# eps696/aphantasia

Hardware: AMD Instinct MI355X
Metric: optimization steps/sec @1280x720 ViT-B/32 samples=200 (higher is better)
Workload: dtype f16 (MFMA operands, fp32 accumulate; fp32 residual stream / LayerNorm / softmax statistics / synth / sampler / loss / Adam)

## Files before the change

### aphantasia_amd/_ffi.py

```python
import ctypes
import os
from ctypes import POINTER, c_char_p, c_float, c_int, c_size_t, c_void_p

import torch

HERE = os.path.dirname(os.path.abspath(__file__))
LIB_PATH = os.path.join(HERE, 'libaphantasia_hip.so')

APH_OUT_NCHW_RAW, APH_OUT_NCHW_NORM, APH_OUT_PATCH_F16, APH_GRAD_PATCH_F16, APH_OUT_PATCH_F16_HILO, APH_OUT_PATCH_F32 = 0, 1, 2, 3, 4, 5
APH_AUG_STRIDE = 16
APH_TF_FAST, APH_TF_CUSTOM, APH_TF_ELASTIC = 0, 1, 2
SIM_TYPES = {'cossim': 0, 'cos': 0, None: 0, 'mix': 1, 'ang': 2, 'dot': 3}


class SampleGeom(ctypes.Structure):
    _fields_ = [(n, c_int) for n in ('H', 'W', 'Hp', 'Wp', 'py0', 'px0', 'S', 'size', 'patch')]


_PROTOTYPES = {
    'aph_version': (c_int, []),
    'aph_last_error': (c_char_p, []),
    'aph_synth_plan_create': (c_int, [c_int, c_int, c_int, POINTER(c_void_p)]),
    'aph_synth_plan_destroy': (c_int, [c_void_p]),
    'aph_synth_fft_fwd': (c_int, [c_void_p, c_void_p, c_void_p, c_void_p, c_float, POINTER(c_float), c_int, c_void_p, c_void_p, c_void_p]),
# ... 5 lines not shown
    'aph_synth_stats': (c_int, [c_void_p, c_void_p, c_void_p]),
    'aph_synth_set_stats': (c_int, [c_void_p, c_void_p, c_void_p]),
    'aph_synth_plan_describe': (c_int, [c_void_p, POINTER(c_int)]),
    'aph_idwt_coarse_levels': (c_int, [POINTER(c_int), POINTER(c_int), c_int, c_int]),
    'aph_rgb_priors_ws_bytes': (c_size_t, []),
    'aph_rgb_sharp': (c_int, [c_void_p, c_int, c_int, c_float, c_void_p, c_void_p, c_void_p, c_void_p]),
    'aph_rgb_priors': (c_int, [c_void_p, c_int, c_int, c_float, c_float, c_float, c_void_p, c_void_p, c_void_p, c_void_p]),
    'aph_cppn_param_count': (c_size_t, [c_int, c_int, c_int]),
    'aph_cppn_ws_bytes': (c_size_t, [c_int, c_int, c_int, c_int, c_int]),
    'aph_cppn_fwd': (c_int, [c_void_p, c_int, c_int, c_int, c_void_p, c_void_p, c_int, c_int, c_void_p, c_void_p, c_void_p]),
    'aph_cppn_bwd': (c_int, [c_void_p, c_int, c_int, c_int, c_void_p, c_void_p, c_int, c_int, c_void_p, c_float, c_void_p, c_void_p, c_void_p, c_void_p]),
    'aph_idwt_level_fwd': (c_int, [c_void_p, c_int, c_int, c_void_p, c_int, c_int, c_int, c_void_p, c_void_p, c_int, c_float, c_void_p, c_void_p]),
    'aph_idwt_fwd': (c_int, [c_void_p, c_void_p, c_void_p, c_void_p, c_void_p, c_int, c_int, c_void_p, c_void_p, c_int, c_void_p, c_void_p]),
    'aph_idwt_bwd': (c_int, [c_void_p, c_void_p, c_void_p, c_void_p, c_int, c_int, c_void_p, c_void_p, c_int, c_void_p, c_void_p, c_void_p, c_void_p]),
    'aph_idwt_level_bwd': (c_int, [c_void_p, c_int, c_int, c_int, c_void_p, c_void_p, c_int, c_float, c_void_p, c_int, c_int, c_void_p, c_void_p]),
    'aph_sample_ws_bytes': (c_size_t, [POINTER(SampleGeom), c_int]),
    'aph_sample_fwd': (c_int, [POINTER(SampleGeom), c_void_p, c_void_p, c_void_p, c_void_p, c_void_p, c_int, c_void_p]),
    'aph_sample_bwd': (c_int, [POINTER(SampleGeom), c_void_p, c_float, c_void_p, c_void_p, c_void_p, c_void_p, c_int, c_void_p]),
    'aph_sample_ws_bytes_tf': (c_size_t, [POINTER(SampleGeom), c_int]),
    'aph_sample_fwd_tf': (c_int, [POINTER(SampleGeom), c_int, c_void_p, c_void_p, c_void_p, c_void_p, c_void_p, c_void_p, c_int, c_void_p]),
    'aph_sample_bwd_tf': (c_int, [POINTER(SampleGeom), c_int, c_void_p, c_float, c_void_p, c_void_p, c_void_p, c_void_p, c_void_p, c_int, c_void_p]),
    'aph_triangle_blur': (c_int, [c_void_p, c_int, c_int, c_int, c_int, c_float, c_float, c_void_p, c_void_p]),
    'aph_resize_bicubic': (c_int, [c_void_p, c_int, c_int, c_int, c_void_p, c_int, c_int, c_void_p]),
    'aph_flip_w': (c_int, [c_void_p, c_void_p, c_int, c_int, c_int, c_void_p, c_void_p]),
    'aph_grid_warp': (c_int, [c_void_p, c_void_p, c_int, c_int, c_int, c_float, c_float, c_float, c_float, c_float, c_void_p, c_void_p, c_void_p]),
    'aph_attn_test': (c_int, [c_void_p, c_void_p, c_void_p, c_void_p, c_void_p, c_void_p, c_int, c_int, c_int, c_int, c_void_p]),
    'aph_attn_f32_test': (c_int, [c_void_p, c_void_p, c_void_p, c_void_p, c_void_p, c_void_p, c_int, c_int, c_int, c_int, c_void_p]),
    'aph_attn_causal_f32_test': (c_int, [c_void_p, c_void_p, c_void_p, c_int, c_int, c_int, c_void_p]),
    'aph_text_create': (c_int, [c_int, c_int, c_int, c_int, c_int, c_int, c_int, POINTER(c_void_p)]),
    'aph_text_destroy': (c_int, [c_void_p]),
    'aph_text_workspace_bytes': (c_size_t, [c_void_p]),
    'aph_text_set_weight': (c_int, [c_void_p, c_char_p, c_void_p, c_size_t]),
    'aph_text_forward': (c_int, [c_void_p, c_void_p, c_int, c_void_p, c_void_p]),
    'aph_lpips_create': (c_int, [POINTER(c_int), c_int, c_int, POINTER(c_void_p)]),
    'aph_lpips_destroy': (c_int, [c_void_p]),
    'aph_lpips_workspace_bytes': (c_size_t, [c_void_p]),
    'aph_lpips_set_weight': (c_int, [c_void_p, c_char_p, c_void_p, c_size_t]),
    'aph_lpips_set_target': (c_int, [c_void_p, c_void_p, c_int, c_int, c_void_p]),
    'aph_lpips_value_grad': (c_int, [c_void_p, c_void_p, c_void_p, c_void_p, c_void_p, c_void_p]),
    'aph_lpips_value_grad_half': (c_int, [c_void_p, c_void_p, c_void_p, c_void_p, c_void_p, c_void_p]),
    'aph_lpips_pack_test': (c_int, [c_void_p, c_int, c_int, c_int, c_void_p, c_size_t]),
    'aph_lpips_conv_test': (c_int, [c_void_p, c_int, c_int, c_int, c_void_p, c_int, c_void_p, c_int, c_void_p, c_void_p, c_void_p, c_int, c_int, c_void_p]),
    'aph_lpips_pool_test': (c_int, [c_void_p, c_int, c_int, c_int, c_void_p, c_void_p, c_void_p, c_void_p]),
    'aph_lpips_head_test': (c_int, [c_void_p, c_void_p, c_void_p, c_int, c_int, c_float, c_void_p, c_void_p, c_void_p, c_void_p, c_void_p]),
    'aph_lpips_resize_test': (c_int, [c_void_p, c_int, c_int, c_void_p, c_int, c_void_p]),
    'aph_depth_create': (c_int, [c_int, c_int, c_int, c_int, POINTER(c_int), POINTER(c_int), c_int, c_int, c_int, c_int, c_int, POINTER(c_void_p)]),
    'aph_depth_destroy': (c_int, [c_void_p]),
    'aph_depth_workspace_bytes': (c_size_t, [c_void_p]),
    'aph_depth_set_weight': (c_int, [c_void_p, c_char_p, c_void_p, c_size_t]),
    'aph_depth_set_pos_embed': (c_int, [c_void_p, c_int, c_int, c_void_p, c_size_t]),
    'aph_depth_forward': (c_int, [c_void_p, c_void_p, c_int, c_int, c_int, c_int, c_void_p, c_void_p]),
    'aph_depth_attn_test': (c_int, [c_void_p, c_void_p, c_int, c_int, c_int, c_void_p]),
    'aph_depth_conv_test': (c_int, [c_void_p, c_int, c_int, c_int, c_void_p, c_int, c_void_p, c_int, c_int, c_void_p, c_void_p, c_int, c_int, c_void_p, c_void_p,
                                    c_void_p]),
    'aph_depth_gemm_test': (c_int, [c_void_p, c_int, c_void_p, c_int, c_int, c_int, c_void_p, c_void_p, c_void_p]),
    'aph_depth_convt_test': (c_int, [c_void_p, c_int, c_int, c_int, c_int, c_void_p, c_int, c_int, c_void_p, c_void_p, c_void_p, c_void_p]),
    'aph_depth_resize_test': (c_int, [c_void_p, c_int, c_int, c_int, c_int, c_void_p, c_int, c_int, c_void_p]),
    'aph_depth_gelu_gemm_test': (c_int, [c_void_p, c_void_p, c_int, c_int, c_int, c_void_p, c_void_p, c_void_p]),
    'aph_frame_affine': (c_int, [c_void_p, c_int, c_int, c_int, POINTER(c_float), c_void_p, c_void_p]),
    'aph_patchify_f16': (c_int, [c_void_p, c_int, c_int, c_int, c_void_p, c_void_p]),
    'aph_patchify_f16_hilo': (c_int, [c_void_p, c_int, c_int, c_int, c_void_p, c_void_p]),
    'aph_patchify_f32': (c_int, [c_void_p, c_int, c_int, c_int, c_void_p, c_void_p]),
    'aph_unpatchify_f32': (c_int, [c_void_p, c_int, c_int, c_int, c_float, c_void_p, c_void_p]),
    'aph_patch_row_elems': (c_int, [c_int]),
    'aph_patchify_f16_win': (c_int, [c_void_p, c_int, c_int, c_int, c_int, c_void_p, c_void_p]),
    'aph_unpatchify_f32_win': (c_int, [c_void_p, c_int, c_int, c_int, c_int, c_float, c_void_p, c_void_p]),
    'aph_vit_create': (c_int, [c_int, c_int, c_int, c_int, c_int, c_int, c_int, POINTER(c_void_p)]),
    'aph_vit_destroy': (c_int, [c_void_p]),
    'aph_vit_workspace_bytes': (c_size_t, [c_void_p]),
    'aph_vit_set_weight': (c_int, [c_void_p, c_char_p, c_void_p, c_size_t]),
    'aph_vit_forward': (c_int, [c_void_p, c_void_p, c_int, c_void_p, c_void_p]),
    'aph_vit_forward_hilo': (c_int, [c_void_p, c_void_p, c_int, c_void_p, c_void_p]),
    'aph_vit_enable_hilo': (c_int, [c_void_p]),
    'aph_vit_enable_f32': (c_int, [c_void_p]),
    'aph_vit_forward_f32': (c_int, [c_void_p, c_void_p, c_int, c_void_p, c_void_p]),
    'aph_vit_backward_f32': (c_int, [c_void_p, c_void_p, c_int, c_void_p, c_float, c_void_p]),
    'aph_vit_backward': (c_int, [c_void_p, c_void_p, c_int, c_void_p, c_float, c_void_p]),
    'aph_vit_backward_h': (c_int, [c_void_p, c_void_p, c_int, c_void_p, c_float, c_void_p]),
    'aph_vit_profile': (c_int, [c_void_p, c_int]),
    'aph_vit_profile_read': (c_int, [c_void_p, c_void_p, c_void_p, c_void_p]),
    'aph_gemm_set_mfma32': (c_int, [c_int]),
    'aph_vit_set_fuse_ln': (c_int, [c_int]),
    'aph_crop_adjoint_set_gather': (c_int, [c_int]),
    'aph_crop_adjoint_set_shape': (c_int, [c_int, c_int, c_int, c_int, c_int]),
    'aph_vit_set_grad_stream_f16': (c_int, [c_int]),
    'aph_gemm_set_ws_min_tiles': (c_int, [c_int]),
    'aph_gemm_set_ws_pgroup': (c_int, [c_int]),
    'aph_gemm_set_rs': (c_int, [c_int]),
    'aph_mfma_rate': (c_int, [c_int, c_int, c_void_p, c_void_p, c_void_p]),
    'aph_gemm_rs_probe': (c_int, [c_void_p, c_void_p, c_int, c_int, c_int, c_void_p, c_int, c_void_p, c_void_p]),
    'aph_gemm_ws_probe': (c_int, [c_void_p, c_void_p, c_int, c_int, c_int, c_void_p, c_void_p, c_void_p, c_int, c_void_p, c_void_p]),
    'aph_gemm_f32_test': (c_int, [c_void_p, c_int, c_int, c_void_p, c_int, c_int, c_int, c_int, c_void_p, c_int, c_void_p, c_void_p, c_int, c_void_p, c_size_t, c_void_p]),
    'aph_gemm_f16': (c_int, [c_void_p, c_void_p, c_int, c_int, c_int, c_void_p, c_void_p]),
    'aph_gemm_f16_ld': (c_int, [c_void_p, c_int, c_void_p, c_int, c_int, c_int, c_int, c_void_p, c_int, c_void_p]),
    'aph_gemm_f16_epi_test': (c_int, [c_void_p, c_int, c_void_p, c_int, c_int, c_int, c_int, c_void_p, c_int, c_void_p, c_void_p, c_void_p, c_float, c_int,
                                      c_int, c_int, c_int, c_void_p, c_size_t, c_int, c_void_p]),
    'aph_ln_test': (c_int, [c_int, c_int, c_int, c_int, c_int, c_int, c_int, c_void_p, c_void_p, c_void_p, c_void_p, c_void_p, c_void_p, c_void_p,
                            c_void_p, c_void_p, c_void_p, c_void_p, c_void_p, c_void_p, c_void_p]),
    'aph_sim_loss': (c_int, [c_void_p, c_int, c_int, c_void_p, c_void_p, POINTER(c_float), c_int, c_int, c_int, c_int, c_int, c_float, c_float, c_void_p, c_void_p, c_void_p, c_void_p]),
    'aph_axpy_f32': (c_int, [c_void_p, c_void_p, c_float, c_size_t, c_void_p]),
    'aph_rgb_to_u8': (c_int, [c_void_p, c_int, c_int, c_float, c_void_p, c_void_p]),
    'aph_linear_head': (c_int, [c_void_p, c_int, c_int, c_void_p, c_float, c_float, c_float, c_float, c_void_p, c_void_p, c_void_p]),
    'aph_comm_unique_id': (c_int, [c_void_p]),
    'aph_comm_init': (c_int, [c_int, c_int, c_void_p, POINTER(c_void_p)]),
    'aph_allreduce_f32': (c_int, [c_void_p, c_void_p, c_size_t, c_void_p]),
    'aph_comm_ranks': (c_int, [c_void_p, POINTER(c_int)]),
    'aph_comm_destroy': (c_int, [c_void_p]),
    'aph_adam_step': (c_int, [c_void_p, c_void_p, c_void_p, c_void_p, c_void_p, c_void_p, c_int, c_size_t, c_void_p]),
    'aph_adam_step_guarded': (c_int, [c_void_p, c_void_p, c_void_p, c_void_p, c_void_p, c_void_p, c_int, c_size_t, c_void_p, c_void_p]),
}

EXPORTS = tuple(_PROTOTYPES)

class Library:

    def __init__(self, path):
        if not os.path.isfile(path):
            raise RuntimeError(
                "aphantasia_amd: HIP library not found at %s -- build it with "
                "`python -c 'import __graft_entry__ as g; g.build()'` (hipcc, gfx950). "
                "There is no CPU fallback." % path)
        self.path = path
        self.cdll = ctypes.CDLL(path)
        for name, (res, args) in _PROTOTYPES.items():
            fn = getattr(self.cdll, name)
            fn.restype = res
            fn.argtypes = args

    def last_error(self):
        return (self.cdll.aph_last_error() or b'').decode(errors='replace')

    def call(self, name, *args):
        rc = getattr(self.cdll, name)(*args)
        if rc < 0:
            raise RuntimeError('%s failed (%d): %s' % (name, rc, self.last_error()))
        return rc


_lib = None


def lib():
    global _lib
    if _lib is None:
        import torch
        if torch.cuda.is_available():
            torch.cuda.init()
            torch.empty(1, device='cuda')
        _lib = Library(LIB_PATH)
    return _lib


def ptr(t):
    return c_void_p(t.data_ptr()) if t is not None else c_void_p(0)


def floats(seq):
    if seq is None:
        return None
    arr = (c_float * len(seq))(*[float(v) for v in seq])
    return arr
```

### aphantasia_amd/csrc/sampler.hip

```cpp
#include <cstring>
#include <cstdlib>
#include <type_traits>

#include "sampler_layout.h"
#include "sampler_crop.h"
#include "sampler_crop_adjoint.h"
#include "sampler_warp.h"
#include "sampler_kornia.h"

namespace aph {

struct Nchw { int s, c, i, j; };
__device__ __forceinline__ Nchw nchw_of(size_t idx, int R) {
  return Nchw{(int)(idx / ((size_t)3 * R * R)), (int)((idx / ((size_t)R * R)) % 3), (int)((idx / R) % R), (int)(idx % R)};
}

__global__ void patchify_kernel(const float* __restrict__ x, half_t* __restrict__ out, int S, int R, int p, int hilo) {
  const size_t n = (size_t)S * 3 * R * R;
  const Layout<APH_OUT_PATCH_F16> L(R, p);
  for (size_t idx = (size_t)blockIdx.x * blockDim.x + threadIdx.x; idx < n; idx += (size_t)gridDim.x * blockDim.x) {
    const Nchw e = nchw_of(idx, R);
    const size_t o = L.index(e.s, e.c, e.i, e.j);
    const half_t h = (half_t)x[idx];
    if (!hilo) { out[o] = h; continue; }
// ... 1 lines not shown
    out[q] = h;
    out[q + L.patch_elems()] = (half_t)(x[idx] - (float)h);
  }
}
__global__ void patchify_f32_kernel(const float* __restrict__ x, float* __restrict__ out, int S, int R, int p) {
  const size_t n = (size_t)S * 3 * R * R;
  for (size_t idx = (size_t)blockIdx.x * blockDim.x + threadIdx.x; idx < n; idx += (size_t)gridDim.x * blockDim.x) {
    const Nchw e = nchw_of(idx, R);
    out[patch_index(e.s, e.c, e.i, e.j, R, p)] = x[idx];
  }
}
__global__ void unpatchify_kernel(const float* __restrict__ g, float* __restrict__ out, int S, int R, int p, float gscale) {
  const size_t n = (size_t)S * 3 * R * R;
  for (size_t idx = (size_t)blockIdx.x * blockDim.x + threadIdx.x; idx < n; idx += (size_t)gridDim.x * blockDim.x) {
    const Nchw e = nchw_of(idx, R);
    out[idx] = g[patch_index(e.s, e.c, e.i, e.j, R, p)] * gscale;
  }
}


__global__ void patchify_win_kernel(const float* __restrict__ x, half_t* __restrict__ out, int S, int Rs, int R, int p, int kp) {
  const int gp = R / p, k3 = 3 * p * p;
  const size_t n = (size_t)S * gp * gp * kp;
  for (size_t idx = (size_t)blockIdx.x * blockDim.x + threadIdx.x; idx < n; idx += (size_t)gridDim.x * blockDim.x) {
    const size_t row = idx / kp;
    const int k = (int)(idx - row * kp);
    float v = 0.f;
    if (k < k3) {
      const int s = (int)(row / ((size_t)gp * gp)), pr = (int)(row - (size_t)s * gp * gp), py = pr / gp, px = pr - py * gp;
      const int pix = k / 3, c = k - pix * 3, iy = pix / p, ix = pix - iy * p;
      v = x[(((size_t)s * 3 + c) * Rs + (py * p + iy)) * Rs + (px * p + ix)];
    }
    out[idx] = (half_t)v;
  }
}
__global__ void unpatchify_win_kernel(const float* __restrict__ g, float* __restrict__ out, int S, int Rs, int R, int p, int kp, float gscale) {
  const int gp = R / p;
  const size_t n = (size_t)S * 3 * Rs * Rs;
  for (size_t idx = (size_t)blockIdx.x * blockDim.x + threadIdx.x; idx < n; idx += (size_t)gridDim.x * blockDim.x) {
    const Nchw e = nchw_of(idx, Rs);
    float v = 0.f;
    if (e.i < R && e.j < R) {
      const int py = e.i / p, px = e.j / p, iy = e.i - py * p, ix = e.j - px * p;
      v = g[(((size_t)e.s * gp + py) * gp + px) * kp + (iy * p + ix) * 3 + e.c] * gscale;
    }
    out[idx] = v;
  }
}

}

using namespace aph;

static Geom to_geom(const aph_sample_geom* g) { return Geom{g->H, g->W, g->Hp, g->Wp, g->py0, g->px0, g->S, g->size, g->patch}; }

static int check_geom(const aph_sample_geom* g, int out_mode, const char* who, int max_mode = 2) {
  if (!g) return aph_fail(APH_ERR_ARG, "%s: null geometry", who);
  if (out_mode == APH_OUT_PATCH_F16_HILO && max_mode == 2) max_mode = APH_OUT_PATCH_F16_HILO;
  if (out_mode == APH_OUT_PATCH_F32) max_mode = APH_OUT_PATCH_F32;
  if (g->S < 1 || g->size < 1 || g->H < 1 || g->W < 1 || g->Hp < g->H || g->Wp < g->W)
    return aph_fail(APH_ERR_ARG, "%s: bad geometry S=%d size=%d H=%d W=%d Hp=%d Wp=%d", who, g->S, g->size, g->H, g->W, g->Hp, g->Wp);
  if (out_mode < 0 || out_mode > max_mode || (out_mode == APH_GRAD_PATCH_F16 && max_mode != APH_GRAD_PATCH_F16))
    return aph_fail(APH_ERR_ARG, "%s: bad out_mode %d", who, out_mode);
  if (out_mode >= APH_OUT_PATCH_F16 && (g->patch < 1 || g->size % g->patch || (g->patch & (g->patch - 1))))
    return aph_fail(APH_ERR_ARG, "%s: size %d not divisible by patch %d, or patch not a power of two", who, g->size, g->patch);
  return APH_OK;
}

namespace {
template <int... MODES> struct Modes {};
template <int... MODES, class F>
bool dispatch_out(Modes<MODES...>, int out_mode, F&& f) {
  return ((out_mode == MODES ? (f(std::integral_constant<int, MODES>{}), true) : false) || ...);
}
using FwdModes = Modes<APH_OUT_NCHW_RAW, APH_OUT_NCHW_NORM, APH_OUT_PATCH_F16, APH_OUT_PATCH_F32, APH_OUT_PATCH_F16_HILO>;
using GradModes = Modes<APH_OUT_NCHW_RAW, APH_OUT_NCHW_NORM, APH_OUT_PATCH_F16, APH_GRAD_PATCH_F16>;

size_t tab_bytes(const Geom& g) {
  const size_t maxcs = (size_t)(g.Hp < g.Wp ? g.Hp : g.Wp);
  return ((size_t)g.S * 2 * maxcs * sizeof(AdjEntry) + 255) & ~(size_t)255;
}
size_t scratch_floats(const Geom& g) { return (size_t)g.S * 4 * g.size * g.size; }
size_t strip_bytes(const Geom& g) { return ((size_t)(8 * (size_t)strip_cap(g) + 8) * sizeof(int) + 255) & ~(size_t)255; }
int* ws_strips(void* ws, const Geom& g) { return reinterpret_cast<int*>(static_cast<char*>(ws) + tab_bytes(g)); }
float* ws_scratch(void* ws, const Geom& g) { return reinterpret_cast<float*>(static_cast<char*>(ws) + tab_bytes(g) + strip_bytes(g)); }
size_t canvas_floats(const Geom& g) { const size_t P = (size_t)g.size + 2 * kTfPad; return (size_t)g.S * 4 * P * P; }

int check_tf(const aph_sample_geom* g, int tf, int out_mode, const float* aug, const float* h_aug, const char* who) {
  if (tf != APH_TF_CUSTOM && tf != APH_TF_ELASTIC) return aph_fail(APH_ERR_ARG, "%s: bad chain kind %d (APH_TF_FAST / _CUSTOM / _ELASTIC)", who, tf);
  if (!aug) return aph_fail(APH_ERR_ARG, "%s: null augment table (the custom / elastic chains draw a rotation and a jitter per cut)", who);
  if (out_mode >= APH_OUT_PATCH_F16 && g->patch <= 2 * kTfPad)
    return aph_fail(APH_ERR_ARG, "%s: patch %d <= 8: the %d x %d canvas holds more than %d patches a side, which the positional embedding of a %d-pixel tower does not cover",
                    who, g->patch, g->size + 2 * kTfPad, g->size + 2 * kTfPad, g->size / g->patch, g->size);
  for (int s = 0; h_aug && s < g->S; ++s) {
    const float dx = h_aug[(size_t)s * APH_AUG_STRIDE], dy = h_aug[(size_t)s * APH_AUG_STRIDE + 1];
    if (!(dx >= 0.f && dx < (float)kTfJitter && dy >= 0.f && dy < (float)kTfJitter && dx == (float)(int)dx && dy == (float)(int)dy))
      return aph_fail(APH_ERR_ARG, "%s: cut %d: jitter (dx, dy) = (%g, %g) outside 0 .. %d", who, s, dx, dy, kTfJitter - 1);
  }
  return APH_OK;
}
}

extern "C" {

int aph_crop_adjoint_set_shape(int rb, int cpt, int nbc, int nseg, int order) {
  CropAdjointShape& v = crop_adjoint_shape();
  v.rb = rb; v.cpt = cpt; v.nbc = nbc; v.nseg = nseg; v.order = order;
  return APH_OK;
}
int aph_crop_adjoint_set_gather(int on) {
  const int prev = crop_adjoint_gather();
  crop_adjoint_gather() = on ? 1 : 0;
  return prev;
}

size_t aph_sample_ws_bytes(const aph_sample_geom* gg, int with_aug) {
  if (!gg || gg->S < 1 || gg->size < 1 || gg->Hp < 1 || gg->Wp < 1) return 0;
  const Geom g = to_geom(gg);
  return tab_bytes(g) + strip_bytes(g) + (with_aug ? 2 * scratch_floats(g) * sizeof(float) : 0);
}

int aph_sample_fwd(const aph_sample_geom* gg, const float* rgb, const int32_t* table_, const float* aug, void* ws,
                   void* out, int out_mode, void* stream_) {
  APH_TRY
  if (int e = check_geom(gg, out_mode, "aph_sample_fwd")) return e;
  if (!rgb || !table_ || !out || !ws) return aph_fail(APH_ERR_ARG, "aph_sample_fwd: null argument (the workspace of aph_sample_ws_bytes is required)");
  hipStream_t st = (hipStream_t)stream_;
  const Geom g = to_geom(gg);
  const int n = g.size;
  const int* table = (const int*)table_;
  int* strips = ws_strips(ws, g);
  if (!aug) {
    if (!dispatch_out(FwdModes{}, out_mode, [&](auto m) { launch_crop_resize<decltype(m)::value>(rgb, table, out, g, strips, st); })) return aph_fail(APH_ERR_ARG, "aph_sample_fwd: no kernel for out_mode %d", out_mode);
    return aph_check_launch("aph_sample_fwd");
  }
  float* A = ws_scratch(ws, g);
  float* Bv = A + scratch_floats(g);
  const dim3 grid((n + 31) / 32, (n + 7) / 8, g.S), block(256);
  launch_crop_resize<APH_SCRATCH_HWC4>(rgb, table, (void*)A, g, strips, st);
  APH_LAUNCH(persp_kernel, grid, block, 0, st, (const float*)A, aug, Bv, n);
  if (!dispatch_out(FwdModes{}, out_mode, [&](auto m) { APH_LAUNCH(rotate_emit_kernel<decltype(m)::value>, grid, block, 0, st, (const float*)A, (const float*)Bv, aug, out, n, g.patch); })) return aph_fail(APH_ERR_ARG, "aph_sample_fwd: no kernel for out_mode %d", out_mode);
  return aph_check_launch("aph_sample_fwd");
  APH_CATCH
}

int aph_sample_bwd(const aph_sample_geom* gg, const void* gout, float gscale, const int32_t* table_, const float* aug,
                   void* ws, float* grgb, int out_mode, void* stream_) {
  APH_TRY
  if (int e = check_geom(gg, out_mode, "aph_sample_bwd", APH_GRAD_PATCH_F16)) return e;
  if (out_mode == APH_OUT_PATCH_F32) out_mode = APH_OUT_PATCH_F16;
  if (!gout || !table_ || !grgb || !ws) return aph_fail(APH_ERR_ARG, "aph_sample_bwd: null argument (the workspace of aph_sample_ws_bytes is required)");
  hipStream_t st = (hipStream_t)stream_;
  const Geom g = to_geom(gg);
  const int n = g.size;
  const int* table = (const int*)table_;
  AdjEntry* tab = static_cast<AdjEntry*>(ws);
  int rc = APH_OK;
  if (!aug) {
    if (!dispatch_out(GradModes{}, out_mode, [&](auto m) { rc = launch_crop_adjoint<decltype(m)::value>(gout, gscale, table, grgb, g, tab, st); })) return aph_fail(APH_ERR_ARG, "aph_sample_bwd: no kernel for out_mode %d", out_mode);
    return rc ? rc : aph_check_launch("aph_sample_bwd");
  }
  float* dA = ws_scratch(ws, g);
  float* dB = dA + scratch_floats(g);
  const dim3 grid((n + 31) / 32, (n + 7) / 8, g.S), block(256);
  if (!dispatch_out(GradModes{}, out_mode, [&](auto m) { APH_LAUNCH(rotate_emit_adjoint_kernel<decltype(m)::value>, grid, block, 0, st, gout, aug, dA, dB, n, g.patch); })) return aph_fail(APH_ERR_ARG, "aph_sample_bwd: no kernel for out_mode %d", out_mode);
  APH_LAUNCH(persp_adjoint_kernel, grid, block, 0, st, (const float*)dB, aug, dA, n);
  rc = launch_crop_adjoint<APH_OUT_NCHW_RAW>((const void*)dA, gscale, table, grgb, g, tab, st);
  return rc ? rc : aph_check_launch("aph_sample_bwd");
  APH_CATCH
}

size_t aph_sample_ws_bytes_tf(const aph_sample_geom* gg, int tf) {
  if (tf == APH_TF_FAST) return aph_sample_ws_bytes(gg, 1);
  if (!gg || gg->S < 1 || gg->size < 1 || gg->Hp < 1 || gg->Wp < 1 || (tf != APH_TF_CUSTOM && tf != APH_TF_ELASTIC)) return 0;
  const Geom g = to_geom(gg);
  return tab_bytes(g) + strip_bytes(g) + (scratch_floats(g) + (tf == APH_TF_ELASTIC ? canvas_floats(g) : 0)) * sizeof(float);
}

int aph_sample_fwd_tf(const aph_sample_geom* gg, int tf, const float* rgb, const int32_t* table_, const float* aug, const float* h_aug,
                      void* ws, void* out, int out_mode, void* stream_) {
  if (tf == APH_TF_FAST) return aph_sample_fwd(gg, rgb, table_, aug, ws, out, out_mode, stream_);
  APH_TRY
  if (int e = check_geom(gg, out_mode, "aph_sample_fwd_tf")) return e;
  if (int e = check_tf(gg, tf, out_mode, aug, h_aug, "aph_sample_fwd_tf")) return e;
  if (!rgb || !table_ || !out || !ws) return aph_fail(APH_ERR_ARG, "aph_sample_fwd_tf: null argument (the workspace of aph_sample_ws_bytes_tf is required)");
  hipStream_t st = (hipStream_t)stream_;
  const Geom g = to_geom(gg);
  const int n = g.size, P = n + 2 * kTfPad, side = out_mode >= APH_OUT_PATCH_F16 ? n : P;
  float* A = ws_scratch(ws, g);
  const dim3 grid((side + 31) / 32, (side + 7) / 8, g.S), block(256);
  launch_crop_resize<APH_SCRATCH_HWC4>(rgb, (const int*)table_, (void*)A, g, ws_strips(ws, g), st);
  bool ok;
  if (tf == APH_TF_CUSTOM) {
    ok = dispatch_out(FwdModes{}, out_mode, [&](auto m) { APH_LAUNCH(custom_emit_kernel<decltype(m)::value>, grid, block, 0, st, (const float*)A, aug, out, n, g.patch); });
  } else {
    ok = dispatch_out(FwdModes{}, out_mode, [&](auto m) { APH_LAUNCH(elastic_emit_kernel<decltype(m)::value>, grid, block, 0, st, (const float*)A, aug, out, n, g.patch); });
  }
  if (!ok) return aph_fail(APH_ERR_ARG, "aph_sample_fwd_tf: no kernel for out_mode %d", out_mode);
  return aph_check_launch("aph_sample_fwd_tf");
  APH_CATCH
}

int aph_sample_bwd_tf(const aph_sample_geom* gg, int tf, const void* gout, float gscale, const int32_t* table_, const float* aug,
                      const float* h_aug, void* ws, float* grgb, int out_mode, void* stream_) {
  if (tf == APH_TF_FAST) return aph_sample_bwd(gg, gout, gscale, table_, aug, ws, grgb, out_mode, stream_);
  APH_TRY
  if (int e = check_geom(gg, out_mode, "aph_sample_bwd_tf", APH_GRAD_PATCH_F16)) return e;
  if (int e = check_tf(gg, tf, out_mode, aug, h_aug, "aph_sample_bwd_tf")) return e;
  if (out_mode == APH_OUT_PATCH_F32) out_mode = APH_OUT_PATCH_F16;
  if (!gout || !table_ || !grgb || !ws) return aph_fail(APH_ERR_ARG, "aph_sample_bwd_tf: null argument (the workspace of aph_sample_ws_bytes_tf is required)");
  hipStream_t st = (hipStream_t)stream_;
  const Geom g = to_geom(gg);
  const int n = g.size, P = n + 2 * kTfPad;
  float* dA = ws_scratch(ws, g);
  float* dB = dA + scratch_floats(g);
  const dim3 grid((n + 31) / 32, (n + 7) / 8, g.S), canvas((P + 31) / 32, (P + 7) / 8, g.S), block(256);
  bool ok;
  if (tf == APH_TF_CUSTOM) {
    ok = dispatch_out(GradModes{}, out_mode, [&](auto m) { APH_LAUNCH(custom_adjoint_kernel<decltype(m)::value>, grid, block, 0, st, gout, aug, dA, n, g.patch); });
  } else {
    ok = dispatch_out(GradModes{}, out_mode, [&](auto m) { APH_LAUNCH(resample_adjoint_kernel<decltype(m)::value>, canvas, block, 0, st, gout, aug, dB, n, g.patch); });
    if (ok) APH_LAUNCH(rotate_canvas_adjoint_kernel, grid, block, 0, st, (const float*)dB, aug, dA, n);
  }
  if (!ok) return aph_fail(APH_ERR_ARG, "aph_sample_bwd_tf: no kernel for out_mode %d", out_mode);
// ... 69 lines not shown
```

### aphantasia_amd/csrc/sampler_crop.h

```cpp
#pragma once
#include "sampler_layout.h"

namespace aph {

__device__ __forceinline__ void bicubic3(const float* __restrict__ rgb, const Geom& g, const CutBox& b, int i, int j, float v[3]) {
  const float sy = src_index(b.scale, i), sx = src_index(b.scale, j);
  const int y0 = (int)floorf(sy), x0 = (int)floorf(sx);
  float wy[4], wx[4];
  cubic_w(sy - (float)y0, wy);
  cubic_w(sx - (float)x0, wx);
  int ry[4], rx[4];
#pragma unroll
  for (int k = 0; k < 4; ++k) {
    int yy = y0 - 1 + k; yy = yy < 0 ? 0 : (yy > b.cs - 1 ? b.cs - 1 : yy);
    int xx = x0 - 1 + k; xx = xx < 0 ? 0 : (xx > b.cs - 1 ? b.cs - 1 : xx);
    ry[k] = wrap(b.oy + yy - g.py0, g.H);
    rx[k] = wrap(b.ox + xx - g.px0, g.W);
  }
  if (wave_all(rx[3] == rx[0] + 3)) {
    F4u t[3][4];
#pragma unroll
    for (int c = 0; c < 3; ++c)
#pragma unroll
      for (int a = 0; a < 4; ++a) t[c][a] = *reinterpret_cast<const F4u*>(rgb + ((size_t)c * g.H + ry[a]) * g.W + rx[0]);
#pragma unroll
    for (int c = 0; c < 3; ++c) {
      float acc = 0.f;
#pragma unroll
      for (int a = 0; a < 4; ++a) acc += (t[c][a].v[0] * wx[0] + t[c][a].v[1] * wx[1] + t[c][a].v[2] * wx[2] + t[c][a].v[3] * wx[3]) * wy[a];
      v[c] = acc;
    }
    return;
  }
#pragma unroll
  for (int c = 0; c < 3; ++c) {
    const float* pl = rgb + (size_t)c * g.H * g.W;
    float acc = 0.f;
#pragma unroll
    for (int a = 0; a < 4; ++a) {
      const float* row = pl + (size_t)ry[a] * g.W;
      acc += (row[rx[0]] * wx[0] + row[rx[1]] * wx[1] + row[rx[2]] * wx[2] + row[rx[3]] * wx[3]) * wy[a];
    }
    v[c] = acc;
  }
}

constexpr int kStripPx = 16;
constexpr int kUnitRows = 4;
constexpr int kStripSlots = 768;

__global__ __launch_bounds__(1024) void strip_list_kernel(const int* __restrict__ table, int* __restrict__ lists, int* __restrict__ counts, int cap, Geom g, int strip_px) {
  __shared__ int cnt[8];
  if (threadIdx.x < 8) cnt[threadIdx.x] = 0;
  __syncthreads();
  const int groups = (g.size + kUnitRows - 1) / kUnitRows, units = g.S * groups;
  for (int u = threadIdx.x; u < units; u += blockDim.x) {
    const int s = u / groups, rg = u - s * groups;
    const CutBox b = load_cut(table, s, g.size);
    int i = rg * kUnitRows + kUnitRows / 2; i = i > g.size - 1 ? g.size - 1 : i;
    int yy = (int)floorf(src_index(b.scale, i)); yy = yy > b.cs - 1 ? b.cs - 1 : yy;
    const int yc = wrap(b.oy + yy - g.py0, g.H);
    const int xcd = (yc / strip_px) & 7;
    const int pos = atomicAdd(&cnt[xcd], 1);
    lists[xcd * cap + pos] = u;
  }
  __syncthreads();
  if (threadIdx.x < 8) counts[threadIdx.x] = cnt[threadIdx.x];
}

template <int OUT>
__global__ __launch_bounds__(256) void crop_resize_strips_kernel(const float* __restrict__ rgb, const int* __restrict__ table, void* __restrict__ out, Geom g,
                                                                 const int* __restrict__ lists, const int* __restrict__ counts, int cap) {
  const int xcd = blockIdx.x & 7, slot = blockIdx.x >> 3, nslot = gridDim.x >> 3;
  const int count = counts[xcd], groups = (g.size + kUnitRows - 1) / kUnitRows, n = g.size;
  for (int it = slot; it < count; it += nslot) {
    const int u = lists[xcd * cap + it];
    const int s = u / groups, rg = u - s * groups;
    const CutBox b = load_cut(table, s, n);
    for (int p = threadIdx.x; p < kUnitRows * n; p += blockDim.x) {
      const int di = p / n, j = p - di * n, i = rg * kUnitRows + di;
      if (i >= n) continue;
      float v[3];
      bicubic3(rgb, g, b, i, j, v);
      emit3<OUT>(out, s, i, j, n, g.patch, v[0], v[1], v[2]);
    }
  }
}

inline int strip_cap(const Geom& g) { return g.S * ((g.size + kUnitRows - 1) / kUnitRows); }

template <int OUT>
void launch_crop_resize(const float* rgb, const int* table, void* out, const Geom& g, int* lists, hipStream_t st) {
  int* counts = lists + 8 * (size_t)strip_cap(g);
  APH_LAUNCH(strip_list_kernel, dim3(1), dim3(1024), 0, st, table, lists, counts, strip_cap(g), g, kStripPx);
  APH_LAUNCH(crop_resize_strips_kernel<OUT>, dim3(8 * kStripSlots), dim3(256), 0, st, rgb, table, out, g, (const int*)lists, (const int*)counts, strip_cap(g));
}

}
```

### aphantasia_amd/csrc/sampler_layout.h

```cpp
#pragma once
#include "aph_device.h"
#include "aph_host.h"

namespace aph {

__device__ __constant__ const float kClipMean[3] = {0.48145466f, 0.4578275f, 0.40821073f};
__device__ __constant__ const float kClipStd[3] = {0.26862954f, 0.26130258f, 0.27577711f};

struct Geom { int H, W, Hp, Wp, py0, px0, S, size, patch; };

__device__ __forceinline__ void cubic_w(float t, float w[4]) {
  const float A = -0.75f;
  const float x1 = t, x2 = 1.0f - t;
  w[0] = ((A * (x1 + 1.0f) - 5.0f * A) * (x1 + 1.0f) + 8.0f * A) * (x1 + 1.0f) - 4.0f * A;
  w[1] = ((A + 2.0f) * x1 - (A + 3.0f)) * x1 * x1 + 1.0f;
  w[2] = ((A + 2.0f) * x2 - (A + 3.0f)) * x2 * x2 + 1.0f;
  w[3] = ((A * (x2 + 1.0f) - 5.0f * A) * (x2 + 1.0f) + 8.0f * A) * (x2 + 1.0f) - 4.0f * A;
}

struct __attribute__((packed, aligned(4))) F4u { float v[4]; };
struct __attribute__((packed, aligned(4))) F3u { float v[3]; };

__device__ __forceinline__ bool wave_all(bool p) {
#ifdef APH_EMU
  return p;
#else
  return __builtin_amdgcn_ballot_w64(!p) == 0;
#endif
}

__device__ __forceinline__ int wrap(int v, int n) {
  if (v < 0) v += n;
  else if (v >= n) v -= n;
  if (v < 0 || v >= n) { v %= n; if (v < 0) v += n; }
  return v;
}

__device__ __forceinline__ float cut_scale(int cs, int size) { return size > 1 ? (float)(cs - 1) / (float)(size - 1) : 0.f; }

__device__ __forceinline__ float src_index(float scale, int i) {
#pragma clang fp contract(off)
  return scale * (float)i;
}

struct CutBox { int cs, ox, oy; float scale; };
__device__ __forceinline__ CutBox load_cut(const int* __restrict__ table, int s, int size) {
  CutBox b;
  b.cs = table[3 * s]; b.ox = table[3 * s + 1]; b.oy = table[3 * s + 2];
  b.scale = cut_scale(b.cs, size);
  return b;
}

template <int OUT>
struct is_patch { static constexpr bool v = OUT == APH_OUT_PATCH_F16 || OUT == APH_GRAD_PATCH_F16; };

template <int OUT>
struct Layout {
  int size, p, lp;
  __device__ __forceinline__ Layout(int size_, int patch) : size(size_), p(patch), lp(is_patch<OUT>::v ? __ffs(patch) - 1 : 0) {}
  __device__ __forceinline__ int patch_elems() const { return 3 << (2 * lp); }
  __device__ __forceinline__ int cut_stride() const { return 3 * size * size; }
  __device__ __forceinline__ int chan_stride() const { return is_patch<OUT>::v ? 1 : size * size; }
  __device__ __forceinline__ int rowpart(int i) const { return is_patch<OUT>::v ? (i >> lp) * (size >> lp) * patch_elems() + ((i & (p - 1)) << lp) * 3 : i * size; }
  __device__ __forceinline__ int colpart(int j) const { return is_patch<OUT>::v ? (j >> lp) * patch_elems() + (j & (p - 1)) * 3 : j; }
  __device__ __forceinline__ int row_of(int off) const {
    if (is_patch<OUT>::v) {
      const int rs = (size >> lp) * patch_elems();
      const int ip = off / rs;
      return (ip << lp) + (off - ip * rs) / (3 << lp);
    }
    return off / size;
  }
  __device__ __forceinline__ int col_of(int off) const {
    if (is_patch<OUT>::v) {
      const int jp = ((off >> (2 * lp)) * 43) >> 7;
      return (jp << lp) + (((off - jp * patch_elems()) * 43) >> 7);
    }
    return off;
  }
  __device__ __forceinline__ size_t index(int s, int c, int i, int j) const {
    return (size_t)s * cut_stride() + (size_t)(rowpart(i) + colpart(j) + c * chan_stride());
  }
  __device__ __forceinline__ size_t hilo_index(size_t o) const { return o + (o / (size_t)patch_elems()) * (size_t)patch_elems(); }
  __device__ __forceinline__ static float load(const void* __restrict__ g, size_t o) {
    return OUT == APH_GRAD_PATCH_F16 ? (float)reinterpret_cast<const half_t*>(g)[o] : reinterpret_cast<const float*>(g)[o];
  }
  __device__ __forceinline__ void load3(const void* __restrict__ g, size_t o, float q[3]) const {
    if (OUT == APH_GRAD_PATCH_F16) {
      const half_t* h = reinterpret_cast<const half_t*>(g) + o;
      q[0] = (float)h[0]; q[1] = (float)h[1]; q[2] = (float)h[2];
    } else if (is_patch<OUT>::v) {
      const F3u t = *reinterpret_cast<const F3u*>(reinterpret_cast<const float*>(g) + o);
      q[0] = t.v[0]; q[1] = t.v[1]; q[2] = t.v[2];
    } else {
      const size_t nn = (size_t)chan_stride();
      q[0] = load(g, o); q[1] = load(g, o + nn); q[2] = load(g, o + 2 * nn);
    }
  }
};

__device__ __forceinline__ size_t patch_index(int s, int c, int i, int j, int size, int p) {
  return Layout<APH_OUT_PATCH_F16>(size, p).index(s, c, i, j);
}

constexpr int APH_SCRATCH_HWC4 = 8;
__device__ __forceinline__ size_t hwc4_index(int s, int i, int j, int size) { return (((size_t)s * size + i) * size + j) * 4; }

template <int OUT>
__device__ __forceinline__ void fetch_grad3(const void* __restrict__ gout, int s, int i, int j, int size, int patch, float g[3]) {
  const Layout<OUT> L(size, patch);
  L.load3(gout, L.index(s, 0, i, j), g);
// ... 38 lines not shown
```

### aphantasia_amd/csrc/sampler_warp.h

```cpp
#pragma once
#include "sampler_layout.h"

namespace aph {

struct Tap { int x0, y0; float wx0, wx1, wy0, wy1; };

__device__ __forceinline__ Tap make_tap(float gx, float gy, int w, int h) {
#pragma clang fp contract(off)
  const float ix = ((gx + 1.f) * (float)w - 1.f) * 0.5f;
  const float iy = ((gy + 1.f) * (float)h - 1.f) * 0.5f;
  Tap t;
  const float fx = floorf(ix), fy = floorf(iy);
  t.x0 = (int)fx; t.y0 = (int)fy;
  t.wx1 = ix - fx; t.wx0 = (fx + 1.f) - ix;
  t.wy1 = iy - fy; t.wy0 = (fy + 1.f) - iy;
  return t;
}
__device__ __forceinline__ Tap make_tap(float gx, float gy, int n) { return make_tap(gx, gy, n, n); }

__device__ __forceinline__ Tap persp_tap(const float* __restrict__ a, int i, int j, int n) {
#pragma clang fp contract(off)
  const float x = (float)j + 0.5f, y = (float)i + 0.5f, hn = 0.5f * (float)n;
  const float g1x = x * (a[0] / hn) + y * (a[1] / hn) + (a[2] / hn);
  const float g1y = x * (a[3] / hn) + y * (a[4] / hn) + (a[5] / hn);
  const float g2 = x * a[6] + y * a[7] + 1.0f;
  return make_tap(g1x / g2 - 1.0f, g1y / g2 - 1.0f, n);
}

__device__ __forceinline__ Tap rot_tap(float cs, float sn, int i, int j, int n) {
#pragma clang fp contract(off)
  const float x = -(float)n * 0.5f + 0.5f + (float)j, y = -(float)n * 0.5f + 0.5f + (float)i, hn = 0.5f * (float)n;
  const float gx = x * (cs / hn) + y * (sn / hn) + (0.0f / hn);
  const float gy = x * (-sn / hn) + y * (cs / hn) + (0.0f / hn);
  return make_tap(gx, gy, n);
}

__device__ __forceinline__ bool in_rect(const float* __restrict__ a, int y, int x) {
  const int eh = (int)a[11];
  if (eh <= 0) return false;
  const int ei = (int)a[9], ej = (int)a[10], ew = (int)a[12];
  return y >= ei && y < ei + eh && x >= ej && x < ej + ew;
}

template <bool ERASE>
__device__ __forceinline__ void warp_gather3(const float* __restrict__ src, const Tap& t, int n, const float* __restrict__ a, float v[3]) {
  float m = 0.f;
  v[0] = v[1] = v[2] = 0.f;
#pragma unroll
  for (int dy = 0; dy < 2; ++dy)
#pragma unroll
    for (int dx = 0; dx < 2; ++dx) {
      const int yy = t.y0 + dy, xx = t.x0 + dx;
      const bool in = yy >= 0 && yy < n && xx >= 0 && xx < n;
      const float w = in ? (dx ? t.wx1 : t.wx0) * (dy ? t.wy1 : t.wy0) : 0.f;
      const int yc = yy < 0 ? 0 : (yy > n - 1 ? n - 1 : yy), xc = xx < 0 ? 0 : (xx > n - 1 ? n - 1 : xx);
      const f32x4 sv = *reinterpret_cast<const f32x4*>(src + ((size_t)yc * n + xc) * 4);
      m += w;
      const float we = (ERASE && in_rect(a, yc, xc)) ? 0.f : w;
      v[0] += we * sv[0]; v[1] += we * sv[1]; v[2] += we * sv[2];
    }
  v[0] *= m; v[1] *= m; v[2] *= m;
}

__global__ void persp_kernel(const float* __restrict__ A, const float* __restrict__ aug, float* __restrict__ Bo, int n) {
  const int s = blockIdx.z;
  const float* a = aug + (size_t)s * APH_AUG_STRIDE;
  if (a[8] == 0.f) return;
  const int j = blockIdx.x * 32 + (threadIdx.x & 31), i = blockIdx.y * 8 + (threadIdx.x >> 5);
  if (i >= n || j >= n) return;
  const Tap t = persp_tap(a, i, j, n);
  float v[3];
  warp_gather3<false>(A + hwc4_index(s, 0, 0, n), t, n, a, v);
  *reinterpret_cast<f32x4*>(Bo + hwc4_index(s, i, j, n)) = f32x4{v[0], v[1], v[2], 0.f};
}

template <int OUT>
__global__ void rotate_emit_kernel(const float* __restrict__ A, const float* __restrict__ Bi, const float* __restrict__ aug,
                                   void* __restrict__ out, int n, int patch) {
  const int s = blockIdx.z;
  const float* a = aug + (size_t)s * APH_AUG_STRIDE;
  const int j = blockIdx.x * 32 + (threadIdx.x & 31), i = blockIdx.y * 8 + (threadIdx.x >> 5);
  if (i >= n || j >= n) return;
  const float* src = (a[8] != 0.f ? Bi : A) + hwc4_index(s, 0, 0, n);
  float v[3];
  if (a[15] != 0.f) {
    const Tap t = rot_tap(a[13], a[14], i, j, n);
    warp_gather3<true>(src, t, n, a, v);
  } else {
    const f32x4 q = *reinterpret_cast<const f32x4*>(src + ((size_t)i * n + j) * 4);
    const bool er = in_rect(a, i, j);
    v[0] = er ? 0.f : q[0]; v[1] = er ? 0.f : q[1]; v[2] = er ? 0.f : q[2];
  }
  emit3<OUT>(out, s, i, j, n, patch, v[0], v[1], v[2]);
}

__device__ __forceinline__ float tap_mask(const Tap& t, int n) {
  float m = 0.f;
  if (t.y0 >= 0 && t.y0 < n) { if (t.x0 >= 0 && t.x0 < n) m += t.wx0 * t.wy0; if (t.x0 + 1 >= 0 && t.x0 + 1 < n) m += t.wx1 * t.wy0; }
  if (t.y0 + 1 >= 0 && t.y0 + 1 < n) { if (t.x0 >= 0 && t.x0 < n) m += t.wx0 * t.wy1; if (t.x0 + 1 >= 0 && t.x0 + 1 < n) m += t.wx1 * t.wy1; }
  return m;
}
__device__ __forceinline__ float tap_hits(const Tap& t, int py, int px) {
  const int dy = py - t.y0, dx = px - t.x0;
  if (dy < 0 || dy > 1 || dx < 0 || dx > 1) return 0.f;
  return (dx ? t.wx1 : t.wx0) * (dy ? t.wy1 : t.wy0);
}

template <int OUT>
__global__ void rotate_emit_adjoint_kernel(const void* __restrict__ gout, const float* __restrict__ aug,
                                           float* __restrict__ dA, float* __restrict__ dB, int n, int patch) {
  const int s = blockIdx.z;
  const float* a = aug + (size_t)s * APH_AUG_STRIDE;
  const int px = blockIdx.x * 32 + (threadIdx.x & 31), py = blockIdx.y * 8 + (threadIdx.x >> 5);
  if (py >= n || px >= n) return;
  float* dst = a[8] != 0.f ? dB : dA;
  float g0 = 0.f, g1 = 0.f, g2 = 0.f;
  if (!in_rect(a, py, px)) {
    if (a[15] != 0.f) {
      const float cs = a[13], sn = a[14], c = 0.5f * (float)(n - 1);
      const float ux = (float)px - c, uy = (float)py - c;
      const float qx = cs * ux - sn * uy + c, qy = sn * ux + cs * uy + c;
      const float rad = fabsf(cs) + fabsf(sn) + 0.02f;
      int j0 = (int)ceilf(qx - rad), j1 = (int)floorf(qx + rad), i0 = (int)ceilf(qy - rad), i1 = (int)floorf(qy + rad);
      if (rad <= 1.45f) {
        const float fn = (float)n, hn = 0.5f * fn, ka = cs / hn, kb = sn / hn;
        const Layout<OUT> L(n, patch);
        float gxj[3], gyj[3], gxi[3], gyi[3];
        size_t rowo[3], colo[3];
        bool iok[3], jok[3];
#pragma unroll
        for (int t = 0; t < 3; ++t) {
#pragma clang fp contract(off)
          const int i = i0 + t, j = j0 + t;
          iok[t] = i >= 0 && i <= n - 1 && i <= i1;
          jok[t] = j >= 0 && j <= n - 1 && j <= j1;
          const int ic = i < 0 ? 0 : (i > n - 1 ? n - 1 : i), jc = j < 0 ? 0 : (j > n - 1 ? n - 1 : j);
          const float x = -fn * 0.5f + 0.5f + (float)jc, y = -fn * 0.5f + 0.5f + (float)ic;
          gxj[t] = x * ka; gyj[t] = x * -kb;
          gxi[t] = y * kb; gyi[t] = y * ka;
          colo[t] = (size_t)L.colpart(jc);
          rowo[t] = (size_t)L.rowpart(ic);
        }
        const size_t base = (size_t)s * L.cut_stride();
        const float fpx = (float)px, fpy = (float)py;
        float wm[9];
        size_t off[9];
#pragma unroll
        for (int d = 0; d < 9; ++d) {
#pragma clang fp contract(off)
          const int a3 = d / 3, b3 = d % 3;
          const float gx = gxj[b3] + gxi[a3], gy = gyj[b3] + gyi[a3];
          const float ix = ((gx + 1.f) * fn - 1.f) * 0.5f, iy = ((gy + 1.f) * fn - 1.f) * 0.5f;
          const float wx = fmaxf(0.f, 1.f - fabsf(ix - fpx)), wy = fmaxf(0.f, 1.f - fabsf(iy - fpy));
          const float mx = fminf(fmaxf(fminf(ix + 1.f, fn - ix), 0.f), 1.f), my = fminf(fmaxf(fminf(iy + 1.f, fn - iy), 0.f), 1.f);
          wm[d] = (iok[a3] && jok[b3]) ? (wx * wy) * (mx * my) : 0.f;
          off[d] = base + rowo[a3] + colo[b3];
        }
        float gv[9][3];
#pragma unroll
        for (int d = 0; d < 9; ++d) L.load3(gout, off[d], gv[d]);
#pragma unroll
        for (int d = 0; d < 9; ++d) { g0 += wm[d] * gv[d][0]; g1 += wm[d] * gv[d][1]; g2 += wm[d] * gv[d][2]; }
        if (OUT != APH_OUT_NCHW_RAW) { g0 /= kClipStd[0]; g1 /= kClipStd[1]; g2 /= kClipStd[2]; }
// ... 96 lines not shown
```

Measured before the change: 176.8.

## Emit non-rotated cuts directly from crop and perspective stages, compact perspective work list

The forward augment chain now writes the final output straight from the crop-resize kernel when a cut has neither perspective nor rotation, and from the perspective kernel when it has no rotation. The rotate/emit kernel then exits early for those cuts. The perspective kernel no longer launches a full grid over every cut: it walks a compacted list of cuts with perspective enabled, built by the strip-list kernel with a ballot. This removes intermediate scratch round-trips and idle blocks, at the cost of more templated code paths, an extra workspace region, and a careful FMA ordering to keep results bitwise-identical.

```diff
diff --git a/aphantasia_amd/_ffi.py b/aphantasia_amd/_ffi.py
--- a/aphantasia_amd/_ffi.py
+++ b/aphantasia_amd/_ffi.py
@@ -111,6 +111,7 @@
     'aph_gemm_set_mfma32': (c_int, [c_int]),
     'aph_vit_set_fuse_ln': (c_int, [c_int]),
     'aph_crop_adjoint_set_gather': (c_int, [c_int]),
+    'aph_sample_set_paths': (c_int, [c_int]),
     'aph_crop_adjoint_set_shape': (c_int, [c_int, c_int, c_int, c_int, c_int]),
     'aph_vit_set_grad_stream_f16': (c_int, [c_int]),
     'aph_gemm_set_ws_min_tiles': (c_int, [c_int]),
diff --git a/aphantasia_amd/csrc/sampler.hip b/aphantasia_amd/csrc/sampler.hip
--- a/aphantasia_amd/csrc/sampler.hip
+++ b/aphantasia_amd/csrc/sampler.hip
@@ -107,9 +107,14 @@
 }
 size_t scratch_floats(const Geom& g) { return (size_t)g.S * 4 * g.size * g.size; }
 size_t strip_bytes(const Geom& g) { return ((size_t)(8 * (size_t)strip_cap(g) + 8) * sizeof(int) + 255) & ~(size_t)255; }
+size_t plist_bytes(const Geom& g) { return (((size_t)g.S + 1) * sizeof(int) + 255) & ~(size_t)255; }
+int* ws_plist(void* ws, const Geom& g) { return reinterpret_cast<int*>(static_cast<char*>(ws) + tab_bytes(g) + strip_bytes(g) + 2 * scratch_floats(g) * sizeof(float)); }
 int* ws_strips(void* ws, const Geom& g) { return reinterpret_cast<int*>(static_cast<char*>(ws) + tab_bytes(g)); }
 float* ws_scratch(void* ws, const Geom& g) { return reinterpret_cast<float*>(static_cast<char*>(ws) + tab_bytes(g) + strip_bytes(g)); }
 size_t canvas_floats(const Geom& g) { const size_t P = (size_t)g.size + 2 * kTfPad; return (size_t)g.S * 4 * P * P; }
+
+enum { kPathClass = 1, kPathList = 2, kPathAll = 15 };
+int& sample_paths() { static int v = kPathAll; return v; }
 
 int check_tf(const aph_sample_geom* g, int tf, int out_mode, const float* aug, const float* h_aug, const char* who) {
   if (tf != APH_TF_CUSTOM && tf != APH_TF_ELASTIC) return aph_fail(APH_ERR_ARG, "%s: bad chain kind %d (APH_TF_FAST / _CUSTOM / _ELASTIC)", who, tf);
@@ -139,10 +144,16 @@
   return prev;
 }
 
+int aph_sample_set_paths(int mask) {
+  const int prev = sample_paths();
+  sample_paths() = mask & kPathAll;
+  return prev;
+}
+
 size_t aph_sample_ws_bytes(const aph_sample_geom* gg, int with_aug) {
   if (!gg || gg->S < 1 || gg->size < 1 || gg->Hp < 1 || gg->Wp < 1) return 0;
   const Geom g = to_geom(gg);
-  return tab_bytes(g) + strip_bytes(g) + (with_aug ? 2 * scratch_floats(g) * sizeof(float) : 0);
+  return tab_bytes(g) + strip_bytes(g) + (with_aug ? 2 * scratch_floats(g) * sizeof(float) + plist_bytes(g) : 0);
 }
 
 int aph_sample_fwd(const aph_sample_geom* gg, const float* rgb, const int32_t* table_, const float* aug, void* ws,
@@ -162,9 +173,15 @@
   float* A = ws_scratch(ws, g);
   float* Bv = A + scratch_floats(g);
   const dim3 grid((n + 31) / 32, (n + 7) / 8, g.S), block(256);
-  launch_crop_resize<APH_SCRATCH_HWC4>(rgb, table, (void*)A, g, strips, st);
-  APH_LAUNCH(persp_kernel, grid, block, 0, st, (const float*)A, aug, Bv, n);
-  if (!dispatch_out(FwdModes{}, out_mode, [&](auto m) { APH_LAUNCH(rotate_emit_kernel<decltype(m)::value>, grid, block, 0, st, (const float*)A, (const float*)Bv, aug, out, n, g.patch); })) return aph_fail(APH_ERR_ARG, "aph_sample_fwd: no kernel for out_mode %d", out_mode);
+  const int paths = sample_paths(), direct = paths & kPathClass;
+  int* plist = ws_plist(ws, g);
+  const FastChain fc{aug, plist, !(paths & kPathList), direct ? out : nullptr};
+  if (!dispatch_out(FwdModes{}, out_mode, [&](auto m) {
+        constexpr int OUT = decltype(m)::value;
+        launch_crop_resize<APH_SCRATCH_HWC4, OUT>(rgb, table, (void*)A, g, strips, st, fc);
+        APH_LAUNCH(persp_kernel<OUT>, dim3(persp_grid(g.S, n)), block, 0, st, (const float*)A, aug, (const int*)plist, Bv, out, n, g.patch, direct);
+        APH_LAUNCH(rotate_emit_kernel<OUT>, grid, block, 0, st, (const float*)A, (const float*)Bv, aug, out, n, g.patch, direct);
+      })) return aph_fail(APH_ERR_ARG, "aph_sample_fwd: no kernel for out_mode %d", out_mode);
   return aph_check_launch("aph_sample_fwd");
   APH_CATCH
 }
diff --git a/aphantasia_amd/csrc/sampler_crop.h b/aphantasia_amd/csrc/sampler_crop.h
--- a/aphantasia_amd/csrc/sampler_crop.h
+++ b/aphantasia_amd/csrc/sampler_crop.h
@@ -1,5 +1,6 @@
 #pragma once
 #include "sampler_layout.h"
+#include "sampler_warp.h"
 
 namespace aph {
 
@@ -49,7 +50,9 @@
 constexpr int kUnitRows = 4;
 constexpr int kStripSlots = 768;
 
-__global__ __launch_bounds__(1024) void strip_list_kernel(const int* __restrict__ table, int* __restrict__ lists, int* __restrict__ counts, int cap, Geom g, int strip_px) {
+__global__ __launch_bounds__(1024) void strip_list_kernel(const int* __restrict__ table, int* __restrict__ lists, int* __restrict__ counts, int cap, Geom g, int strip_px,
+                                                          const float* __restrict__ aug, int* __restrict__ plist, int every) {
+  if (plist && threadIdx.x >= blockDim.x - 64) write_persp_list(aug, g.S, plist, every);
   __shared__ int cnt[8];
   if (threadIdx.x < 8) cnt[threadIdx.x] = 0;
   __syncthreads();
@@ -68,32 +71,43 @@
   if (threadIdx.x < 8) counts[threadIdx.x] = cnt[threadIdx.x];
 }
 
-template <int OUT>
+template <int OUT, int FIN>
 __global__ __launch_bounds__(256) void crop_resize_strips_kernel(const float* __restrict__ rgb, const int* __restrict__ table, void* __restrict__ out, Geom g,
-                                                                 const int* __restrict__ lists, const int* __restrict__ counts, int cap) {
+                                                                 const int* __restrict__ lists, const int* __restrict__ counts, int cap,
+                                                                 const float* __restrict__ aug, void* __restrict__ fin) {
   const int xcd = blockIdx.x & 7, slot = blockIdx.x >> 3, nslot = gridDim.x >> 3;
   const int count = counts[xcd], groups = (g.size + kUnitRows - 1) / kUnitRows, n = g.size;
   for (int it = slot; it < count; it += nslot) {
     const int u = lists[xcd * cap + it];
     const int s = u / groups, rg = u - s * groups;
     const CutBox b = load_cut(table, s, n);
+    const float* a = aug ? aug + (size_t)s * APH_AUG_STRIDE : nullptr;
+    const bool finish = a && a[8] == 0.f && a[15] == 0.f;
     for (int p = threadIdx.x; p < kUnitRows * n; p += blockDim.x) {
       const int di = p / n, j = p - di * n, i = rg * kUnitRows + di;
       if (i >= n) continue;
       float v[3];
       bicubic3(rgb, g, b, i, j, v);
-      emit3<OUT>(out, s, i, j, n, g.patch, v[0], v[1], v[2]);
+      if (finish) {
+        const bool er = in_rect(a, i, j);
+        emit3<FIN>(fin, s, i, j, n, g.patch, er ? 0.f : rounded(v[0]), er ? 0.f : rounded(v[1]), er ? 0.f : rounded(v[2]));
+      } else {
+        emit3<OUT>(out, s, i, j, n, g.patch, v[0], v[1], v[2]);
+      }
     }
   }
 }
 
 inline int strip_cap(const Geom& g) { return g.S * ((g.size + kUnitRows - 1) / kUnitRows); }
 
-template <int OUT>
-void launch_crop_resize(const float* rgb, const int* table, void* out, const Geom& g, int* lists, hipStream_t st) {
+struct FastChain { const float* aug = nullptr; int* plist = nullptr; int every = 0; void* fin = nullptr; };
+
+template <int OUT, int FIN = OUT>
+void launch_crop_resize(const float* rgb, const int* table, void* out, const Geom& g, int* lists, hipStream_t st, const FastChain& fc = FastChain{}) {
   int* counts = lists + 8 * (size_t)strip_cap(g);
-  APH_LAUNCH(strip_list_kernel, dim3(1), dim3(1024), 0, st, table, lists, counts, strip_cap(g), g, kStripPx);
-  APH_LAUNCH(crop_resize_strips_kernel<OUT>, dim3(8 * kStripSlots), dim3(256), 0, st, rgb, table, out, g, (const int*)lists, (const int*)counts, strip_cap(g));
+  APH_LAUNCH(strip_list_kernel, dim3(1), dim3(1024), 0, st, table, lists, counts, strip_cap(g), g, kStripPx, fc.aug, fc.plist, fc.every);
+  APH_LAUNCH((crop_resize_strips_kernel<OUT, FIN>), dim3(8 * kStripSlots), dim3(256), 0, st, rgb, table, out, g, (const int*)lists, (const int*)counts, strip_cap(g),
+             fc.fin ? fc.aug : nullptr, fc.fin);
 }
 
 }
diff --git a/aphantasia_amd/csrc/sampler_layout.h b/aphantasia_amd/csrc/sampler_layout.h
--- a/aphantasia_amd/csrc/sampler_layout.h
+++ b/aphantasia_amd/csrc/sampler_layout.h
@@ -27,6 +27,13 @@
 #else
   return __builtin_amdgcn_ballot_w64(!p) == 0;
 #endif
+}
+
+__device__ __forceinline__ float rounded(float x) {
+#ifndef APH_EMU
+  asm volatile("" : "+v"(x));
+#endif
+  return x;
 }
 
 __device__ __forceinline__ int wrap(int v, int n) {
diff --git a/aphantasia_amd/csrc/sampler_warp.h b/aphantasia_amd/csrc/sampler_warp.h
--- a/aphantasia_amd/csrc/sampler_warp.h
+++ b/aphantasia_amd/csrc/sampler_warp.h
@@ -62,23 +62,83 @@
   v[0] *= m; v[1] *= m; v[2] *= m;
 }
 
-__global__ void persp_kernel(const float* __restrict__ A, const float* __restrict__ aug, float* __restrict__ Bo, int n) {
+__device__ __forceinline__ void persp_gather3(const float* __restrict__ src, const Tap& t, int n, float v[3]) {
+  float w[4];
+  f32x4 sv[4];
+#pragma unroll
+  for (int k = 0; k < 4; ++k) {
+#pragma clang fp contract(off)
+    const int dy = k >> 1, dx = k & 1, yy = t.y0 + dy, xx = t.x0 + dx;
+    const bool in = yy >= 0 && yy < n && xx >= 0 && xx < n;
+    w[k] = in ? (dx ? t.wx1 : t.wx0) * (dy ? t.wy1 : t.wy0) : 0.f;
+    const int yc = yy < 0 ? 0 : (yy > n - 1 ? n - 1 : yy), xc = xx < 0 ? 0 : (xx > n - 1 ? n - 1 : xx);
+    sv[k] = *reinterpret_cast<const f32x4*>(src + ((size_t)yc * n + xc) * 4);
+  }
+  const float c0 = fmaf(w[3], sv[3][0], fmaf(w[2], sv[2][0], fmaf(w[1], sv[1][0], fmaf(w[0], sv[0][0], 0.f))));
+  const float c1 = fmaf(w[3], sv[3][1], fmaf(w[2], sv[2][1], fmaf(w[1], sv[1][1], fmaf(w[0], sv[0][1], 0.f))));
+  const float c2 = fmaf(w[2], sv[2][2], fmaf(w[1], sv[1][2], fmaf(w[0], sv[0][2], 0.f)));
+  {
+#pragma clang fp contract(off)
+    const float m = (((0.f + w[0]) + w[1]) + w[2]) + w[3];
+    const float last = w[3] * sv[3][2];
+    v[0] = c0 * m; v[1] = c1 * m; v[2] = (last + c2) * m;
+  }
+}
+
+__device__ __forceinline__ void write_persp_list(const float* __restrict__ aug, int S, int* __restrict__ plist, int every) {
+  const int lane = threadIdx.x & 63;
+  int count = 0;
+  for (int base = 0; base < S; base += 64) {
+    const int s = base + lane;
+    const bool on = s < S && (every || aug[(size_t)s * APH_AUG_STRIDE + 8] != 0.f);
+    const unsigned long long m = __ballot(on);
+    if (on) plist[1 + count + __popcll(m & ((1ull << lane) - 1ull))] = s;
+    count += __popcll(m);
+  }
+  if (lane == 0) plist[0] = count;
+}
+
+constexpr int kPerspGrid = 2048;
+inline int persp_tiles(int n) { return ((n + 31) / 32) * ((n + 7) / 8); }
+inline int persp_grid(int S, int n) { const long long t = (long long)S * persp_tiles(n); return (int)(t < kPerspGrid ? t : kPerspGrid); }
+struct PerspUnit { int s, i, j; bool on; };
+__device__ __forceinline__ PerspUnit persp_unit(const float* __restrict__ aug, const int* __restrict__ plist, int w, int n) {
+  const int tx = (n + 31) / 32, tiles = tx * ((n + 7) / 8);
+  const int c = w / tiles, tile = w - c * tiles, ty = tile / tx;
+  PerspUnit u;
+  u.s = plist[1 + c];
+  u.j = (tile - ty * tx) * 32 + (threadIdx.x & 31);
+  u.i = ty * 8 + (threadIdx.x >> 5);
+  u.on = aug[(size_t)u.s * APH_AUG_STRIDE + 8] != 0.f && u.i < n && u.j < n;
+  return u;
+}
+
+template <int OUT>
+__global__ __launch_bounds__(256) void persp_kernel(const float* __restrict__ A, const float* __restrict__ aug, const int* __restrict__ plist,
+                                                    float* __restrict__ Bo, void* __restrict__ out, int n, int patch, int direct) {
+  const int total = plist[0] * (((n + 31) / 32) * ((n + 7) / 8));
+  for (int w = blockIdx.x; w < total; w += gridDim.x) {
+    const PerspUnit u = persp_unit(aug, plist, w, n);
+    if (!u.on) continue;
+    const float* a = aug + (size_t)u.s * APH_AUG_STRIDE;
+    const Tap t = persp_tap(a, u.i, u.j, n);
+    float v[3];
+    persp_gather3(A + hwc4_index(u.s, 0, 0, n), t, n, v);
+    if (direct && a[15] == 0.f) {
+      const bool er = in_rect(a, u.i, u.j);
+      emit3<OUT>(out, u.s, u.i, u.j, n, patch, er ? 0.f : rounded(v[0]), er ? 0.f : rounded(v[1]), er ? 0.f : rounded(v[2]));
+    } else {
+      *reinterpret_cast<f32x4*>(Bo + hwc4_index(u.s, u.i, u.j, n)) = f32x4{v[0], v[1], v[2], 0.f};
+    }
+  }
+}
+
+template <int OUT>
+__global__ void rotate_emit_kernel(const float* __restrict__ A, const float* __restrict__ Bi, const float* __restrict__ aug,
+                                   void* __restrict__ out, int n, int patch, int direct) {
   const int s = blockIdx.z;
   const float* a = aug + (size_t)s * APH_AUG_STRIDE;
-  if (a[8] == 0.f) return;
-  const int j = blockIdx.x * 32 + (threadIdx.x & 31), i = blockIdx.y * 8 + (threadIdx.x >> 5);
-  if (i >= n || j >= n) return;
-  const Tap t = persp_tap(a, i, j, n);
-  float v[3];
-  warp_gather3<false>(A + hwc4_index(s, 0, 0, n), t, n, a, v);
-  *reinterpret_cast<f32x4*>(Bo + hwc4_index(s, i, j, n)) = f32x4{v[0], v[1], v[2], 0.f};
-}
-
-template <int OUT>
-__global__ void rotate_emit_kernel(const float* __restrict__ A, const float* __restrict__ Bi, const float* __restrict__ aug,
-                                   void* __restrict__ out, int n, int patch) {
-  const int s = blockIdx.z;
-  const float* a = aug + (size_t)s * APH_AUG_STRIDE;
+  if (direct && a[15] == 0.f) return;
   const int j = blockIdx.x * 32 + (threadIdx.x & 31), i = blockIdx.y * 8 + (threadIdx.x >> 5);
   if (i >= n || j >= n) return;
   const float* src = (a[8] != 0.f ? Bi : A) + hwc4_index(s, 0, 0, n);
```

New measurement: 176.8 (median of 2 runs). No clear change (+0.0%).
